# gonewest818/raytrace-clj

Hardware: AMD Instinct MI355X
Metric: Msamples/sec (nx*ny*ns) (higher is better)
Workload: dtype f64; 1 GPU; C3: 1920x1080x256spp Shirley cover scene n=50 (10001 spheres), depth 50, thin-lens camera, seeded counter RNG; accel=bvh; 8x8 tiles dealt round-robin to 1 GPU(s); nx=1920, ny=1080, ns=256, spheres=10001, depth=50, accel=bvh, accel_ran=bvh, frames_in_flight=1, launch_form=one GPU

## Files before the change

include/rtmi.h:

```cpp
#ifndef RTMI_H
#define RTMI_H

#include <stdint.h>

#ifdef __cplusplus
extern "C" {
#endif

#define RTMI_OK 0
#define RTMI_E_ARG (-1)
#define RTMI_E_DEVICE (-2)
#define RTMI_E_UNSUPPORTED (-3)
#define RTMI_E_NOMEM (-4)
#define RTMI_E_STATE (-5)

enum { RTMI_PRIM_SPHERE = 0, RTMI_PRIM_UVSPHERE = 1, RTMI_PRIM_MOVING = 2,
       RTMI_PRIM_RECT_XY = 3, RTMI_PRIM_RECT_XZ = 4, RTMI_PRIM_RECT_YZ = 5, RTMI_PRIM_TRIANGLE = 6,
       RTMI_PRIM_MEDIUM = 7, RTMI_PRIM_BOUNDARY = 16 };
enum { RTMI_XFORM_TRANSLATE = 0, RTMI_XFORM_ROTATE_Y = 1 };
enum { RTMI_MAT_LAMBERTIAN = 0, RTMI_MAT_METAL = 1, RTMI_MAT_DIELECTRIC = 2, RTMI_MAT_DIFFUSE_LIGHT = 3,
       RTMI_MAT_ISOTROPIC = 4  };
enum { RTMI_TEX_CONSTANT = 0, RTMI_TEX_UVGRADIENT = 1, RTMI_TEX_CHECKER = 2,
       RTMI_TEX_PERLIN_NOISE = 3, RTMI_TEX_PERLIN_TURB = 4, RTMI_TEX_MARBLE = 5, RTMI_TEX_FLIP_U = 6, RTMI_TEX_FLIP_V = 7,
       RTMI_TEX_IMAGE = 8 };
// ... 146 lines not shown
int rtmi_last_accel(rtmi_ctx *ctx, int32_t *accel);
int rtmi_last_gather_ms(rtmi_ctx *ctx0, double *ms);

int rtmi_last_traversal_counters(rtmi_ctx *ctx, uint64_t *out_aabb_tests, uint64_t *out_prim_tests);

int rtmi_last_trace_ms(rtmi_ctx *ctx, double *ms, int32_t *launches);
int rtmi_last_reduce_ms(rtmi_ctx *ctx, double *ms, int32_t *launches);

int rtmi_probe_hit(rtmi_scene *scene, int32_t precision, int32_t n, const double *rays, double t_min, double t_max, double *out);
int rtmi_probe_paths(rtmi_scene *scene, int32_t precision, int32_t n, const double *rays, const uint64_t *keys, uint64_t ctr0,
                     int32_t depth, double *out_rgb, uint64_t *out_nseg, double *log, int32_t max_seg, int32_t *out_nlog);
int rtmi_probe_camera(rtmi_scene *scene, int32_t precision, int32_t n, const double *uv, const uint64_t *keys, double *out);
int rtmi_probe_texture(rtmi_scene *scene, int32_t precision, int32_t tex, int32_t n, const double *uvp, double *out);
int rtmi_probe_scatter(rtmi_scene *scene, int32_t precision, int32_t mat, int32_t n, const double *rays, const double *hits,
                       const uint64_t *keys, double *out);
int rtmi_probe_rng(rtmi_ctx *ctx, int32_t precision, uint64_t key, uint64_t d0, int32_t n, uint64_t *out_bits, double *out_real);
uint64_t rtmi_sample_key(uint64_t seed, uint64_t pixel, uint64_t sample);
int rtmi_probe_arith(rtmi_ctx *ctx, int32_t n, const double *abc, double *out);
#define RTMI_PROBE_MATH_SLOTS 12
int rtmi_probe_math2(rtmi_ctx *ctx, int32_t n, const double *abc, double tmin, double tmax, int32_t n_slots, double *out);
int rtmi_probe_math(rtmi_ctx *ctx, int32_t n, const double *abc, double tmin, double tmax, double *out);

int rtmi_test_build_tree(int32_t n, const double *geom, const double *cam, int32_t threads, uint64_t *out_hash, int32_t *out_info, double *out_ms);
int rtmi_test_half_outward(double x, int32_t up);
int rtmi_test_pack_materials(int32_t n_prims, const int32_t *prim_kind, const double *prim_geom, const int32_t *prim_mat,
                             int32_t n_mats, const int32_t *mat_kind, const int32_t *mat_tex, const double *mat_param,
                             int32_t n_tex, const int32_t *tex_kind, const double *tex_param, const int32_t *tex_child,
                             int32_t cam_kind, const double *cam, const int32_t *prim_flip, const int32_t *prim_xform,
                             int32_t n_xforms, const int32_t *xform_kind, const double *xform_param, int32_t through_creation,
                             uint64_t *out_hash, int32_t *out_facts);
int rtmi_test_pack_geometry(int32_t n_prims, const int32_t *prim_kind, const double *prim_geom, const int32_t *prim_mat,
                            int32_t n_mats, const int32_t *mat_kind, const int32_t *mat_tex, const double *mat_param,
                            int32_t n_tex, const int32_t *tex_kind, const double *tex_param, const int32_t *tex_child,
                            int32_t cam_kind, const double *cam, const int32_t *prim_flip, const int32_t *prim_xform,
                            int32_t n_xforms, const int32_t *xform_kind, const double *xform_param, int32_t through_creation, uint64_t *out_hash);
int rtmi_test_refit(int32_t n_prims, const int32_t *prim_kind, const int32_t *prim_flip, const int32_t *prim_xform, int32_t n_xforms, const int32_t *xform_kind,
                    int32_t cam_kind, const double *cam, int32_t n_steps, const double *geoms, const double *xforms,
                    void *out_nodes, int64_t capacity, int64_t *out_bytes, int32_t *out_info, int32_t *out_big,
                    int32_t *out_cells, int64_t cells_capacity, void *out_leaf_box);
int rtmi_test_refit_half(double x, int32_t up);
int rtmi_test_scene_nodes(rtmi_scene *scene, void *buf, int64_t capacity, int64_t *out_bytes);

#ifdef __cplusplus
}
#endif
#endif
// ... 1 lines not shown
```

raytrace_clj_amd/_ffi.py:

```python
import ctypes as C
import os

import numpy as np

try:
    import torch
except ImportError:
    torch = None

_HERE = os.path.dirname(os.path.abspath(__file__))
LIB_PATH = os.environ.get("RTMI_LIB") or os.path.join(_HERE, "lib", "librtmi.so")

SYMBOLS = [
    "rtmi_last_error", "rtmi_backend_name", "rtmi_version", "rtmi_init", "rtmi_shutdown", "rtmi_set_option",
    "rtmi_device_info", "rtmi_scene_create", "rtmi_scene_create_ex", "rtmi_scene_set_perlin", "rtmi_scene_set_images", "rtmi_scene_set_media_calls", "rtmi_scene_set_media_mode", "rtmi_scene_set_media_calls_narrowed", "rtmi_scene_device_bytes", "rtmi_scene_destroy", "rtmi_render", "rtmi_render_device",
    "rtmi_render_tiles_device", "rtmi_local_tiles", "rtmi_assemble_device", "rtmi_last_trace_ms", "rtmi_last_reduce_ms", "rtmi_probe_hit",
    "rtmi_probe_paths", "rtmi_probe_camera", "rtmi_probe_texture", "rtmi_probe_scatter", "rtmi_probe_rng",
    "rtmi_sample_key", "rtmi_test_half_outward", "rtmi_test_build_tree", "rtmi_probe_arith", "rtmi_probe_math", "rtmi_probe_math2", "rtmi_last_traversal_counters",
    "rtmi_scene_clone", "rtmi_render_multi", "rtmi_render_multi_device", "rtmi_last_gather_ms",
    "rtmi_last_gather_path", "rtmi_rccl_probe", "rtmi_stream_idle", "rtmi_last_passes", "rtmi_last_accel",
    "rtmi_render_progressive", "rtmi_render_progressive_device", "rtmi_progressive_samples", "rtmi_progressive_release",
    "rtmi_render_adaptive", "rtmi_render_adaptive_device", "rtmi_adaptive_status", "rtmi_adaptive_active_tiles",
    "rtmi_render_features", "rtmi_render_features_device", "rtmi_denoise", "rtmi_denoise_device",
    "rtmi_adaptive_retire", "rtmi_adaptive_retire_device",
    "rtmi_render_adaptive_tiles_device", "rtmi_assemble_progressive_device", "rtmi_render_multi_adaptive", "rtmi_render_multi_adaptive_device",
    "rtmi_scene_set_camera", "rtmi_scene_set_camera_stream", "rtmi_scene_camera",
    "rtmi_reproject", "rtmi_reproject_device",
    "rtmi_scene_tree_info",
    "rtmi_scene_set_materials", "rtmi_scene_set_materials_stream", "rtmi_test_pack_materials",
    "rtmi_scene_set_geometry", "rtmi_scene_last_refit_ms", "rtmi_test_pack_geometry", "rtmi_test_refit", "rtmi_test_refit_half", "rtmi_test_scene_nodes",
]

F64, F32 = 0, 1
ACCEL_FLAT, ACCEL_BVH = 0, 1
FLAG_TIMING = 1
GATHER_PATHS = {0: "none", 1: "same-device", 2: "peer-copy", 3: "rccl"}
SEG_REC = 12
TILE = 8
PROG_REC = 5
FEATURES = 8
EDIT_STREAM_MAX_BYTES = 32768
# ... 32 lines not shown
    L.rtmi_scene_set_media_mode.argtypes = [vp, i32]
    L.rtmi_scene_set_media_calls_narrowed.argtypes = [vp, i32, vp, vp]
    L.rtmi_scene_device_bytes.argtypes = [vp, C.POINTER(C.c_int64)]
    L.rtmi_scene_destroy.argtypes = [vp]
    L.rtmi_render.argtypes = [vp, i32, i32, i32, i32, u64, i32, i32, i32, i32, i32, vp, vp, vp]
    L.rtmi_render_device.argtypes = [vp, i32, i32, i32, i32, u64, i32, vp, vp, vp, vp]
    L.rtmi_render_tiles_device.argtypes = [vp, i32, i32, i32, i32, u64, i32, i32, i32, vp, vp, vp]
    L.rtmi_local_tiles.argtypes = [i32, i32, i32, i32]
    L.rtmi_local_tiles.restype = i32
    L.rtmi_assemble_device.argtypes = [vp, i32, i32, i32, i32, vp, vp, vp, vp]
    L.rtmi_last_trace_ms.argtypes = [vp, C.POINTER(dbl), C.POINTER(i32)]
    L.rtmi_last_reduce_ms.argtypes = [vp, C.POINTER(dbl), C.POINTER(i32)]
    L.rtmi_probe_hit.argtypes = [vp, i32, i32, vp, dbl, dbl, vp]
    L.rtmi_probe_paths.argtypes = [vp, i32, i32, vp, vp, u64, i32, vp, vp, vp, i32, vp]
    L.rtmi_probe_camera.argtypes = [vp, i32, i32, vp, vp, vp]
    L.rtmi_probe_texture.argtypes = [vp, i32, i32, i32, vp, vp]
    L.rtmi_probe_scatter.argtypes = [vp, i32, i32, i32, vp, vp, vp, vp]
    L.rtmi_probe_rng.argtypes = [vp, i32, u64, u64, i32, vp, vp]
    L.rtmi_sample_key.argtypes = [u64, u64, u64]
    L.rtmi_sample_key.restype = u64
    L.rtmi_probe_arith.argtypes = [vp, i32, vp, vp]
    L.rtmi_test_build_tree.argtypes = [i32, vp, vp, i32, vp, vp, vp]
    L.rtmi_test_half_outward.argtypes = [C.c_double, i32]
    L.rtmi_probe_math.argtypes = [vp, i32, vp, C.c_double, C.c_double, vp]
    L.rtmi_probe_math2.argtypes = [vp, i32, vp, C.c_double, C.c_double, i32, vp]
    L.rtmi_last_traversal_counters.argtypes = [vp, C.POINTER(u64), C.POINTER(u64)]
    L.rtmi_scene_clone.argtypes = [vp, vp, C.POINTER(vp)]
    L.rtmi_render_multi.argtypes = [i32, C.POINTER(vp), i32, i32, i32, i32, u64, i32, vp, vp, vp]
    L.rtmi_render_multi_device.argtypes = [i32, C.POINTER(vp), i32, i32, i32, i32, u64, i32, vp, vp, vp]
    L.rtmi_last_gather_ms.argtypes = [vp, C.POINTER(dbl)]
    L.rtmi_last_gather_path.argtypes = [vp, C.POINTER(i32)]
    L.rtmi_rccl_probe.argtypes = [C.c_char_p]
    L.rtmi_stream_idle.argtypes = [vp, C.POINTER(i32)]
    L.rtmi_last_passes.argtypes = [vp, C.POINTER(i32)]
    L.rtmi_last_accel.argtypes = [vp, C.POINTER(i32)]
    L.rtmi_render_progressive.argtypes = [vp, i32, i32, i32, i32, i32, u64, i32, i32, i32, i32, i32, vp, vp, vp, vp]
    L.rtmi_render_progressive_device.argtypes = [vp, i32, i32, i32, i32, i32, u64, i32, vp, vp, vp, vp, vp]
    L.rtmi_progressive_samples.argtypes = [vp, C.POINTER(i32)]
    L.rtmi_progressive_release.argtypes = [vp]
    L.rtmi_render_adaptive.argtypes = [vp, i32, i32, i32, i32, dbl, i32, u64, i32, i32, i32, i32, i32, vp, vp, vp, vp, vp]
    L.rtmi_render_adaptive_device.argtypes = [vp, i32, i32, i32, i32, dbl, i32, u64, i32, vp, vp, vp, vp, vp, vp]
    L.rtmi_adaptive_status.argtypes = [vp, C.POINTER(i32), C.POINTER(i32), C.POINTER(i64)]
    L.rtmi_adaptive_active_tiles.argtypes = [vp, i32, vp, C.POINTER(i32)]
    L.rtmi_adaptive_retire.argtypes = [vp, i32, i32, vp, dbl, C.POINTER(i32)]
    L.rtmi_adaptive_retire_device.argtypes = [vp, i32, i32, vp, dbl, C.POINTER(i32), vp]
    L.rtmi_render_features.argtypes =[vp, i32, i32, i32, u64, i32, i32, i32, i32, i32, vp, vp]
# ... 46 lines not shown
```

raytrace_clj_amd/csrc/rtmi.hip:

```cpp
#include <hip/hip_runtime.h>
#include <rccl/rccl.h>
#include <dlfcn.h>

#include <algorithm>
#include <atomic>
#include <chrono>
#include <condition_variable>
#include <functional>
#include <thread>
#include <cmath>
#include <cmath>
#include <cstdarg>
#include <cstdio>
#include <cstdlib>
#include <cstring>
#include <array>
#include <map>
#include <mutex>
#include <new>
#include <string>
#include <vector>

#include "rtmi.h"
#include "rtmi_device.h"
// ... 24 lines not shown
#ifndef RTMI_EXT_MIN_WAVES
#define RTMI_EXT_MIN_WAVES RTMI_MIN_WAVES
#endif

struct TraceParams {
    int nx, ny, depth;
    u64 seed;
    int tiles_x;
    int n_local_tiles;
    const int *tile_ids;
    int s_begin, s_count;
    void *samples;
    u64 *counters;
    int prims_per_tile;
    int n_ptiles;
    unsigned *queue;
    unsigned total_items;
    unsigned qblock;
    int suspend_lanes;
    int rx0, ry0, rx1, ry1;
    u64 *trav;
    int susp_off;
    int stash_off;
};
#ifndef RTMI_QUEUE_BLOCK
#define RTMI_QUEUE_BLOCK 256
#endif
#ifndef RTMI_EXT_NO_STASH
#define RTMI_EXT_NO_STASH 0
#endif
#ifndef RTMI_EXT_LDS_STASH
#define RTMI_EXT_LDS_STASH 1
#endif
#ifndef RTMI_STASH
#define RTMI_STASH 1
#endif
constexpr unsigned kQueueBlock = RTMI_QUEUE_BLOCK;

template <typename R> __device__ inline const R *stat4_of(SceneRef sc);
template <typename R> __device__ inline void stage_prims(SceneRef sc, Prim4<R> *lds, int first, int count) {
    for (int i = threadIdx.x; i < count; i += blockDim.x) {
        const R *g = stat4_of<R>(sc) + (size_t)(first + i) * 4;
        Prim4<R> p;
        p.cx = g[0]; p.cy = g[1]; p.cz = g[2]; p.r2 = g[3];
        lds[i] = p;
    }
// ... 118 lines not shown
            __syncthreads();
            stage_prims<R>(sc, lds, first, count);
            __syncthreads();
            if (active) {
                if (VARIANT == SCAN_LDS_PIPE) scan_static_pipe<R, true>(LdsPrims<R>{lds}, count, first, P, a, tmin, best_t, best_i);
                else scan_static<R>(lds, count, first, P, a, tmin, best_t, best_i);
            }
        }
    }
    if (active) {
        if (best_i >= 0) best_i = sc.stat_orig[best_i];
        if (sc.n_moving > 0) {
            int best_orig = best_i >= 0 ? best_i : 0x7fffffff, scan_i = -1;
            scan_moving<R>(sc, P, a, tmin, best_t, scan_i, best_orig);
            if (scan_i >= 0) best_i = best_orig;
        }
    }
}

template <typename R> __device__ inline void start_sample(SceneRef sc, const TraceParams &tp, int i, int j, int s, Path<R> &P) {
    seed_stream(P, sample_key(tp.seed, (u64)j * (u64)tp.nx + (u64)i, (u64)s), 0u);
    const R u = ((R)(float)i + next_uniform(P)) / (R)tp.nx;
    const R v = ((R)(float)j + next_uniform(P)) / (R)tp.ny;
    get_ray<R>(sc, u, v, P);
    P.ar = P.ag = P.ab = R(1);
    P.depth = tp.depth;
}

template <typename R, bool MULTI, int VARIANT, bool EXT = false, bool COUNT = false, bool SLICE = true, int MSEQ = 0, bool LST = false>
__global__ void __launch_bounds__(kTraceBlock, EXT ? ((MSEQ != 0 || COUNT) ? 3 : RTMI_EXT_MIN_WAVES) : RTMI_MIN_WAVES) trace_kernel(ScenePtr scp, TraceParams tp) {
    SceneRef sc = *scp;
    extern __shared__ __attribute__((aligned(16))) char smem[];
    Prim4<R> *lds = reinterpret_cast<Prim4<R> *>(smem);
    const int lane = threadIdx.x & 63;
    if (!MULTI && VARIANT < SCAN_SGPR) stage_prims<R>(sc, lds, 0, sc.n_static);
    __syncthreads();

    const unsigned total_items = tp.total_items;
    unsigned w_cur = 0, w_end = 0;
    Path<R> P;
    P.ox = P.oy = P.oz = P.dx = P.dy = P.dz = P.time = R(0);
    P.ar = P.ag = P.ab = R(0);
    seed_stream(P, 0ull, 0u); P.depth = 0;
    bool alive = false;
    bool exhausted = (total_items == 0);
    unsigned out_item = 0;
    constexpr bool LSTASH = (EXT && RTMI_STASH && RTMI_EXT_LDS_STASH && !RTMI_EXT_NO_STASH) || LST;
    constexpr bool STASH = RTMI_STASH && !(EXT && RTMI_EXT_NO_STASH) && !LSTASH;
    int *const lst = reinterpret_cast<int *>(smem) + tp.stash_off + (threadIdx.x & ~63);
    R st_ox = R(0), st_oy = R(0), st_oz = R(0), st_dx = R(0), st_dy = R(0), st_dz = R(0), st_time = R(0);
    u64 st_rs = 0;
    unsigned st_item = 0xffffffffu;
    unsigned s_head = 64u;
    unsigned nrays = 0;
    unsigned ntrav[2] = {0u, 0u};
    const R tmin = R(0.001), tmax = Real<R>::tmax();
    constexpr bool SLICED = SLICE && VARIANT == SCAN_BVH && !MULTI;
    bool mid = false;

    RTMI_STAMP_DECL
    for (;;) {
        RTMI_PH(PH_LOOP)
        if (LSTASH) {
        for (;;) {
            const u64 dead = __ballot(!alive);
            if (dead == 0) break;
            if (s_head == 64u) {
                if (exhausted) break;
                if (w_cur == w_end) {
                    unsigned base = 0;
                    if (lane == 0) base = atomicAdd(tp.queue, tp.qblock);
                    base = __builtin_amdgcn_readfirstlane(base);
                    if (base >= total_items) { exhausted = true; break; }
                    w_cur = base;
                    w_end = min(base + tp.qblock, total_items);
                }
                const unsigned m = w_cur + (unsigned)lane;
                w_cur += 64u;
                const unsigned chunk = m >> 6;
                const int l = (int)(m & 63u);
                const int tile_local = (int)(chunk / (unsigned)tp.s_count);
                const int s = tp.s_begin + (int)(chunk - (unsigned)tile_local * (unsigned)tp.s_count);
                const int gtile = tp.tile_ids[tile_local];
                const int x = (gtile % tp.tiles_x) * RTMI_TILE + (l & 7);
                const int y = (gtile / tp.tiles_x) * RTMI_TILE + (l >> 3);
                unsigned item = 0xffffffffu;
                if (x >= tp.rx0 && x < tp.rx1 && y >= tp.ry0 && y < tp.ry1) {
                    Path<R> Q;
                    start_sample<R>(sc, tp, x, tp.ny - 1 - y, s, Q);
                    int w0, w1;
                    best_to_words<R>(Q.dx, w0, w1); lst[lane] = w0; lst[kTraceBlock + lane] = w1;
                    best_to_words<R>(Q.dy, w0, w1); lst[2 * kTraceBlock + lane] = w0; lst[3 * kTraceBlock + lane] = w1;
                    best_to_words<R>(Q.dz, w0, w1); lst[4 * kTraceBlock + lane] = w0; lst[5 * kTraceBlock + lane] = w1;
                    best_to_words<R>(Q.time, w0, w1); lst[6 * kTraceBlock + lane] = w0; lst[7 * kTraceBlock + lane] = w1;
                    lst[8 * kTraceBlock + lane] = (int)(unsigned)Q.rs; lst[9 * kTraceBlock + lane] = (int)(unsigned)(Q.rs >> 32);
                    if (!sc.cam_fixed_origin) {
                        best_to_words<R>(Q.ox, w0, w1); lst[11 * kTraceBlock + lane] = w0; lst[12 * kTraceBlock + lane] = w1;
                        best_to_words<R>(Q.oy, w0, w1); lst[13 * kTraceBlock + lane] = w0; lst[14 * kTraceBlock + lane] = w1;
                        best_to_words<R>(Q.oz, w0, w1); lst[15 * kTraceBlock + lane] = w0; lst[16 * kTraceBlock + lane] = w1;
                    }
                    item = m;
                    RTMI_PH(PH_REFILL_GEN)
                }
                lst[10 * kTraceBlock + lane] = (int)item;
                s_head = 0u;
            }
            const unsigned avail = 64u - s_head, nd = (unsigned)__popcll(dead);
            const unsigned rank = (unsigned)__popcll(dead & ((1ull << lane) - 1ull));
            if (!alive && rank < avail) {
                const int e = (int)(s_head + rank);
                const unsigned item = (unsigned)lst[10 * kTraceBlock + e];
                if (item != 0xffffffffu) {
// ... 8 lines not shown
                    P.ar = P.ag = P.ab = R(1);
                    P.depth = tp.depth;
                    out_item = item;
                    alive = true;
                }
            }
            s_head += min(nd, avail);
        }
        } else if (STASH) {
        for (;;) {
            const u64 dead = __ballot(!alive);
            if (dead == 0) break;
            if (s_head == 64u) {
                if (exhausted) break;
                if (w_cur == w_end) {
                    unsigned base = 0;
                    if (lane == 0) base = atomicAdd(tp.queue, tp.qblock);
                    base = __builtin_amdgcn_readfirstlane(base);
                    if (base >= total_items) { exhausted = true; break; }
                    w_cur = base;
                    w_end = min(base + tp.qblock, total_items);
                }
                const unsigned m = w_cur + (unsigned)lane;
                w_cur += 64u;
                const unsigned chunk = m >> 6;
                const int l = (int)(m & 63u);
                const int tile_local = (int)(chunk / (unsigned)tp.s_count);
                const int s = tp.s_begin + (int)(chunk - (unsigned)tile_local * (unsigned)tp.s_count);
                const int gtile = tp.tile_ids[tile_local];
                const int x = (gtile % tp.tiles_x) * RTMI_TILE + (l & 7);
                const int y = (gtile / tp.tiles_x) * RTMI_TILE + (l >> 3);
                st_item = 0xffffffffu;
                if (x >= tp.rx0 && x < tp.rx1 && y >= tp.ry0 && y < tp.ry1) {
                    Path<R> Q;
                    start_sample<R>(sc, tp, x, tp.ny - 1 - y, s, Q);
                    st_ox = Q.ox; st_oy = Q.oy; st_oz = Q.oz; st_dx = Q.dx; st_dy = Q.dy; st_dz = Q.dz; st_time = Q.time; st_rs = Q.rs;
                    st_item = m;
                    RTMI_PH(PH_REFILL_GEN)
                }
                s_head = 0u;
            }
            const unsigned avail = 64u - s_head, nd = (unsigned)__popcll(dead);
            const unsigned rank = (unsigned)__popcll(dead & ((1ull << lane) - 1ull));
            const bool take = !alive && rank < avail;
            const int src = take ? (int)(s_head + rank) : lane;
            R f_ox, f_oy, f_oz;
            if (sc.cam_fixed_origin) { f_ox = (R)sc.cam[0]; f_oy = (R)sc.cam[1]; f_oz = (R)sc.cam[2]; }
            else { f_ox = __shfl(st_ox, src); f_oy = __shfl(st_oy, src); f_oz = __shfl(st_oz, src); }
            const R f_dx = __shfl(st_dx, src), f_dy = __shfl(st_dy, src), f_dz = __shfl(st_dz, src), f_time = __shfl(st_time, src);
            const u64 f_rs = __shfl(st_rs, src);
            const unsigned f_item = __shfl(st_item, src);
            if (take && f_item != 0xffffffffu) {
                P.ox = f_ox; P.oy = f_oy; P.oz = f_oz; P.dx = f_dx; P.dy = f_dy; P.dz = f_dz; P.time = f_time; P.rs = f_rs;
                P.ar = P.ag = P.ab = R(1);
                P.depth = tp.depth;
                out_item = f_item;
                alive = true;
            }
// ... 1067 lines not shown
                                          : (multi ? trace_kernel<R, true, SCAN_LDS_LITERAL> : trace_kernel<R, false, SCAN_LDS_LITERAL>);
        p.lds.bytes = lds_bytes;
    }
    return p;
}

#ifdef RTMI_STAMPS
int report_phase_stamps(rtmi_ctx *c, hipStream_t st) {
    const int grid_trace_dbg = c->last_grid;
    HIP_TRY(hipStreamSynchronize(st));
    unsigned long long h[3 * PH_SLOTS] = {0}, z[3 * PH_SLOTS] = {0};
    HIP_TRY(hipMemcpyFromSymbol(h, HIP_SYMBOL(g_phase), sizeof(h)));
    HIP_TRY(hipMemcpyToSymbol(HIP_SYMBOL(g_phase), z, sizeof(z)));
    {
        static unsigned long long wt[2][4096];
        HIP_TRY(hipMemcpyFromSymbol(wt, HIP_SYMBOL(g_wg_t), sizeof(wt)));
        const int g = std::min(4096, grid_trace_dbg);
        unsigned long long t0 = ~0ull; for (int k = 0; k < g; ++k) t0 = std::min(t0, wt[0][k]);
        std::vector<double> e(g), b(g); for (int k = 0; k < g; ++k) { e[k] = (wt[1][k] - t0) * 1e-5; b[k] = (wt[0][k] - t0) * 1e-5; }
        std::sort(e.begin(), e.end()); std::sort(b.begin(), b.end());
        fprintf(stderr, "[stamps] workgroup start (ms after first): median %.3f max %.3f | end: min %.3f p10 %.3f median %.3f p90 %.3f max %.3f (last pass, %d workgroups)\n",
                b[g / 2], b[g - 1], e[0], e[g / 10], e[g / 2], e[g * 9 / 10], e[g - 1], g);
    }
    static const char *names[PH_N] = {"loop/tail", "refill: generate 64 camera rays", "refill: claim + deal", "bvh: ray setup / resume", "bvh: big primitives (exact)",
                                      "bvh: descent (node visits)", "bvh: leaf exact tests", "bvh: loop control / park", "shade: hit record", "shade: |d| normalise",
                                      "shade: rand-in-unit-sphere", "shade: material record + directions", "shade: texture", "shade: store / rest", "shade: sphere uv", "(stamp calibration)",
                                      "bvh: grid entry / next piece of the walk", "media: chords, draws, log"};
    const double per_stamp = h[2 * PH_SLOTS + PH_CAL] ? (double)h[PH_CAL] / (double)h[2 * PH_SLOTS + PH_CAL] : 0.0;
    double tk[PH_N], lk[PH_N], tot = 0, totl = 0, raw = 0;
    for (int k = 0; k < PH_N; ++k) {
        raw += (double)h[k];
        const double t = (double)h[k], c = std::min(t, per_stamp * (double)h[2 * PH_SLOTS + k]);
        tk[k] = k == PH_CAL ? 0.0 : t - c;
        lk[k] = t > 0 ? (double)h[PH_SLOTS + k] * (tk[k] / t) : 0.0;
        tot += tk[k]; totl += lk[k];
    }
    fprintf(stderr, "[phases] one stamp = %.0f ticks; stamps took %.1f %% of the %.4g wave-ticks of this (diagnostic) launch and are subtracted below\n", per_stamp, 100 * (raw - tot) / raw, raw);
    fprintf(stderr, "[phases] %-36s %8s %8s %10s %10s %12s\n", "phase", "ticks %", "lanes", "masked %", "useful %", "stamps");
    for (int k = 0; k < PH_N; ++k) {
        if (!h[k] || k == PH_CAL) continue;
        const double t = tk[k], l = lk[k];
        fprintf(stderr, "[phases] %-36s %8.2f %8.1f %10.2f %10.2f %12llu\n", names[k], 100 * t / tot, t > 0 ? l / t : 0.0, 100 * (64 * t - l) / (64 * tot), 100 * l / (64 * tot), h[2 * PH_SLOTS + k]);
    }
    fprintf(stderr, "[phases] %-36s %8.2f %8.1f %10.2f %10.2f   (%.4g wave-ticks)\n", "total", 100.0, totl / tot, 100 * (64 * tot - totl) / (64 * tot), 100 * totl / (64 * tot), tot);
    return RTMI_OK;
}
#endif

template <typename F> auto with_real(int precision, F f) { return precision == RTMI_F64 ? f(double{}) : f(float{}); }

// ... 178 lines not shown
    if (rc) return rc;
    c->last_passes = (ns + s_per_pass - 1) / s_per_pass;
    if (!prog && s_per_pass < ns) {
        rc = c->accum.ensure((size_t)n_local * 64 * 3 * sizeof(R));
        if (rc) return rc;
    }
    int ppt, nptiles;
    size_t lds_bytes;
    lds_plan(c, s->dev.n_static, sizeof(R), &ppt, &nptiles, &lds_bytes);
    const TracePlan plan = choose_trace_kernel<R>(s, c, read_launch_knobs(), nptiles > 1, lds_bytes);
    c->last_accel = plan.accel;

    TraceParams tp;
    tp.nx = nx; tp.ny = ny; tp.depth = depth; tp.seed = seed; tp.tiles_x = tiles_x_of(nx);
    tp.n_local_tiles = n_local;
    tp.tile_ids = ad ? reinterpret_cast<const int *>(prog->act_tiles[prog->cur].p) : reinterpret_cast<const int *>(c->tile_ids.p);
    tp.samples = c->samples.p;
    tp.counters = d_counters ? reinterpret_cast<u64 *>(d_counters) : reinterpret_cast<u64 *>(c->counters.p);
    tp.prims_per_tile = (c->scan_variant >= SCAN_SGPR || s->dev.has_ext) ? 0 : ppt; tp.n_ptiles = nptiles;
    tp.queue = reinterpret_cast<unsigned *>(reinterpret_cast<u64 *>(c->counters.p) + 2);
    tp.rx0 = region.x0; tp.ry0 = region.y0; tp.rx1 = region.x1; tp.ry1 = region.y1;
    tp.trav = reinterpret_cast<u64 *>(c->counters.p) + 3;
    tp.suspend_lanes = plan.suspend_lanes; tp.susp_off = plan.lds.susp_off; tp.stash_off = plan.lds.stash_off;
    for (int s_begin = s_first; s_begin < s_end; s_begin += s_per_pass) {
        hipEvent_t e1 = nullptr;
        rc = launch_trace_pass(s, plan, tp, s_begin, std::min(s_per_pass, s_end - s_begin), st, &e1);
        if (!rc) rc = launch_fold<R>(c, tp, ns, s_end, d_tiles_linear, d_counters != nullptr, prog, ad, e1, st);
        if (rc) return rc;
    }
#ifdef RTMI_STAMPS
    rc = report_phase_stamps(c, st);
#endif
    if (!rc && ad)
        HIP_TRY(launch_compact(*prog, nullptr, n_local, -1, tiles_x_of(nx), region, st));
    if (!rc && prog) prog->k = s_end;
    return rc;
}

template <typename R>
int render_tiles_impl(rtmi_scene *s, int nx, int ny, int ns, int depth, uint64_t seed, int first, int stride, const int *rg, void *d_tiles_linear,
                      void *d_counters, hipStream_t st) {
    return render_passes<R>(s, nx, ny, 0, ns, depth, seed, first, stride, rg, d_tiles_linear, d_counters, st, nullptr);
}

int check_render_args(rtmi_scene *s, int nx, int ny, int ns, int depth, int precision) {
    if (!scene_ok(s)) return fail(RTMI_E_STATE, "invalid scene handle");
// ... 45 lines not shown
    std::vector<int> kind((size_t)n, RTMI_PRIM_SPHERE);
    std::vector<BvhBox> wbox((size_t)n);
    std::vector<char> bounded((size_t)n, 0), box_first((size_t)n, 0);
    for (int i = 0; i < n; ++i) {
        const double g[9] = {geom[4 * (size_t)i], geom[4 * (size_t)i + 1], geom[4 * (size_t)i + 2], geom[4 * (size_t)i + 3], 0, 0, 0, 0, 1};
        bounded[(size_t)i] = prim_world_box(RTMI_PRIM_SPHERE, g, nullptr, nullptr, 0, 0, 0.0, 1.0, wbox[(size_t)i]);
    }
    DevScene d{};
    std::vector<int> grid_cells;
    int depth = 0;
    g_build_single.store(threads == 1 ? 1 : 0);
    const double t0 = now_ms();
    const std::vector<float> nodes = build_bvh(d, n, kind.data(), wbox, bounded, cam, true, grid_cells, box_first, knobs, &depth);
    *out_ms = now_ms() - t0;
    g_build_single.store(0);
    uint64_t h = 1469598103934665603ull;
    auto mix = [&](const void *p, size_t bytes) { const unsigned char *q = (const unsigned char *)p; for (size_t k = 0; k < bytes; ++k) { h ^= q[k]; h *= 1099511628211ull; } };
    mix(nodes.data(), nodes.size() * sizeof(float));
    mix(grid_cells.data(), grid_cells.size() * sizeof(int));
    mix(&d.bvh_root, sizeof(int)); mix(&d.grid_tall, sizeof(int)); mix(&d.bvh_node16, sizeof(int));
    *out_hash = h;
    out_info[0] = (int32_t)(nodes.size() / (d.bvh_node16 ? 8 : 16)); out_info[1] = depth; out_info[2] = d.grid_n; out_info[3] = d.n_big;
    return RTMI_OK;
}
RTMI_EXPORT int rtmi_test_half_outward(double x, int32_t up) { return (int)half_outward((float)x, up != 0); }
RTMI_EXPORT const char *rtmi_last_error(void) { return g_err.c_str(); }
RTMI_EXPORT const char *rtmi_backend_name(void) { return "hip-gfx950"; }
RTMI_EXPORT int rtmi_version(void) { return 214; }
RTMI_EXPORT uint64_t rtmi_sample_key(uint64_t seed, uint64_t pixel, uint64_t sample) { return sample_key(seed, pixel, sample); }

RTMI_EXPORT int rtmi_init(int device, uint32_t flags, rtmi_ctx **out_ctx) {
    if (!out_ctx) return fail(RTMI_E_ARG, "out_ctx is NULL");
    *out_ctx = nullptr;
    int ndev = 0;
    if (hipGetDeviceCount(&ndev) != hipSuccess || ndev <= 0) return fail(RTMI_E_DEVICE, "no HIP device visible (this library has no CPU fallback)");
    if (device < 0 || device >= ndev) return fail(RTMI_E_ARG, "device %d out of range (0..%d)", device, ndev - 1);
    HIP_TRY(hipSetDevice(device));
    hipDeviceProp_t prop;
    HIP_TRY(hipGetDeviceProperties(&prop, device));
    if (std::strncmp(prop.gcnArchName, "gfx950", 6) != 0)
        return fail(RTMI_E_DEVICE, "device %d is %s; this library carries gfx950 (MI355X) code objects only", device, prop.gcnArchName);
    rtmi_ctx *c = new (std::nothrow) rtmi_ctx();
    if (!c) return fail(RTMI_E_NOMEM, "out of host memory");
    c->device = device;
    c->flags = flags;
    c->cus = prop.multiProcessorCount;
// ... 2529 lines not shown
```

raytrace_clj_amd/csrc/rtmi_device.h:

```cpp
#pragma once
#include <hip/hip_runtime.h>
#include <stdint.h>

#include "rtmi.h"

namespace rtmi {

typedef unsigned long long u64;

struct DevScene {
    int n_static;
    int n_moving;
    const double *stat_geom;
    const double *stat4_d;
    const float *stat4_f;
    int n_all;
    const float *cull20;
    const double *exact12;
    double cull_t_lo, cull_t_hi;
    const float *bvh_nodes;
    int bvh_root;
    int n_big;
    int big_idx[16];
    int bvh_node16;
// ... 45 lines not shown
    const int *tex_kind;
    const double *tex_param;
    const int *tex_child;
    int cam_kind;
    int cam_fixed_origin;
    double cam[24];
};
typedef const __attribute__((address_space(4))) DevScene &SceneRef;
typedef const __attribute__((address_space(4))) DevScene *ScenePtr;

#define RTMI_GOLD 0x9E3779B97F4A7C15ULL
__host__ __device__ inline u64 mix64(u64 z) {
    z ^= z >> 32; z *= 0xD6E8FEB86659FD93ULL;
    z ^= z >> 32; z *= 0xD6E8FEB86659FD93ULL;
    z ^= z >> 32;
    return z;
}
__host__ __device__ inline u64 sample_key(u64 seed, u64 pix, u64 s) {
    return mix64(mix64(seed ^ (RTMI_GOLD * (pix + 1))) + 0xD1B54A32D192ED03ULL * (s + 1));
}
__host__ __device__ inline u64 draw_bits(u64 key, u64 d) { return mix64(key + RTMI_GOLD * (d + 1)); }

#ifdef RTMI_STAMPS
enum { PH_LOOP = 0, PH_REFILL_GEN, PH_REFILL_DEAL, PH_BVH_SETUP, PH_BIG, PH_DESCENT, PH_LEAF, PH_BVH_POST, PH_HITREC, PH_DNORM, PH_SAMPLER, PH_DIRS, PH_TEXTURE, PH_STORE, PH_UV, PH_CAL, PH_GRID, PH_MEDIA, PH_N };
#define PH_SLOTS 20
__shared__ unsigned long long g_ph[4][3 * PH_SLOTS + 2];
__device__ inline void ph_stamp(int k, unsigned lane_trips = 0, unsigned trips = 0) {
    __builtin_amdgcn_sched_barrier(0);
    unsigned long long t;
    asm volatile("s_memtime %0\n\ts_waitcnt lgkmcnt(0)" : "=s"(t)::"memory");
    const unsigned long long ex = __ballot(1);
    const int w = threadIdx.x >> 6;
    if ((int)(threadIdx.x & 63) == __ffsll((long long)ex) - 1) {
        const unsigned long long dt = t - g_ph[w][3 * PH_SLOTS];
        if (k >= 0) {
            g_ph[w][2 * PH_SLOTS + k] += 1;
            g_ph[w][k] += dt;
            g_ph[w][PH_SLOTS + k] += trips ? dt * (unsigned long long)lane_trips / (unsigned long long)trips : dt * (unsigned long long)__popcll(ex);
        }
        g_ph[w][3 * PH_SLOTS] = t;
    }
    __builtin_amdgcn_sched_barrier(0);
}
#define RTMI_PH(k) ph_stamp(k);
#define RTMI_PH_LANES(k, lt, tr) ph_stamp(k, lt, tr);
#elif defined(RTMI_MARKERS)
#define RTMI_PH(k) asm volatile("; PHASE_END " #k);
#define RTMI_PH_LANES(k, lt, tr) asm volatile("; PHASE_END " #k);
// ... 247 lines not shown
        const u64 sm = kStrideMask[n];
        const u64 mine = pending ? ((acc >> vrank) & sm) : 0ull;
        const int first = mine ? __ffsll((long long)mine) - 1 : 0;
        const int src = mine ? vrank + first : lane;
        const R fx = __shfl(cx, src), fy = __shfl(cy, src), fz = __shfl(cz, src);
        if (pending) {
            const unsigned used = mine ? 3u * (unsigned)(__popcll(sm & ((1ull << first) - 1ull)) + 1) : 3u * (unsigned)K;
            P.rs += RTMI_GOLD * (u64)used;
            P.ctr += used;
            if (mine) { x = fx; y = fy; z = fz; pending = false; }
        }
        RTMI_PH(PH_SAMPLER)
        rem = __ballot(pending);
    }
#else
    if (need) rand_in_unit_sphere(P, x, y, z);
#endif
}

template <typename R> __device__ inline void rand_in_unit_disk(Path<R> &P, R &x, R &y) {
    for (;;) {
        x = next_symmetric(P);
        y = next_symmetric(P);
        if (!(dot3(x, y, R(0), x, y, R(0)) >= R(1.0))) return;
    }
}

template <typename R> __device__ inline void get_ray(SceneRef sc, R s, R t, Path<R> &P) {
    unsigned long long cam_addr = (unsigned long long)(&sc.cam[0]);
    asm volatile("" : "+s"(cam_addr));
    const __attribute__((address_space(4))) double *c = (const __attribute__((address_space(4))) double *)cam_addr;
    const R ox = (R)c[0], oy = (R)c[1], oz = (R)c[2];
    R dx = (((R)c[3] + (R)c[6] * s) + (R)c[9] * t) + (-ox);
    R dy = (((R)c[4] + (R)c[7] * s) + (R)c[10] * t) + (-oy);
    R dz = (((R)c[5] + (R)c[8] * s) + (R)c[11] * t) + (-oz);
    if (sc.cam_kind == RTMI_CAM_PINHOLE) {
        P.ox = ox; P.oy = oy; P.oz = oz; P.dx = dx; P.dy = dy; P.dz = dz; P.time = R(0);
        return;
    }
    const R lens_radius = (R)c[21] / R(2.0);
    R rx, ry;
    rand_in_unit_disk(P, rx, ry);
    rx = lens_radius * rx; ry = lens_radius * ry;
    const R offx = (R)c[12] * rx + (R)c[15] * ry;
    const R offy = (R)c[13] * rx + (R)c[16] * ry;
    const R offz = (R)c[14] * rx + (R)c[17] * ry;
    P.ox = ox + offx; P.oy = oy + offy; P.oz = oz + offz;
    P.dx = dx + (-offx); P.dy = dy + (-offy); P.dz = dz + (-offz);
    const R t0 = (R)c[22], t1 = (R)c[23];
    P.time = t0 + (t1 - t0) * next_uniform(P);
}

template <typename R> __device__ inline int sin_sign(R x) {
    const R s = Real<R>::sin_(x);
    return s < R(0) ? -1 : (s > R(0) ? 1 : 0);
}
template <> __device__ inline int sin_sign<double>(double x) {
    if (x == 0.0) return 0;
    if (!(fabs(x) <= 1.0e5)) { const double s = ::sin(x); return s < 0.0 ? -1 : (s > 0.0 ? 1 : 0); }
    const double k = ::rint(x * 0.3183098861837907);
    double r = ::fma(-k, 3.141592653589793, x);
    r = ::fma(-k, 1.2246467991473532e-16, r);
    const bool odd = ((int)k) & 1;
    return (odd != (r < 0.0)) ? -1 : 1;
}

template <typename R> __device__ inline R perlin_noise(SceneRef sc, R px, R py, R pz) {
    const R fi = (R)::floor((double)px), fj = (R)::floor((double)py), fk = (R)::floor((double)pz);
    const int i = (int)fi, j = (int)fj, k = (int)fk;
    const R u = px - fi, v = py - fj, w = pz - fk;
    const R uu = (u * u) * (R(3.0) - R(2.0) * u), vv = (v * v) * (R(3.0) - R(2.0) * v), ww = (w * w) * (R(3.0) - R(2.0) * w);
    R acc = R(0);
#pragma unroll
// ... 1461 lines not shown
```

raytrace_clj_amd/csrc/scene_build.h:

```cpp
#pragma once
#include <unistd.h>

namespace {

struct BuildKnobs {
    int sah_levels = 1 << 20;
    int sweep_max = 0;
    double min_frac = 0.0;
    bool grid_off = false;
    int grid_side = 0;
    int grid_kmax = 4;
    bool grid_walk = true;
    bool mloc = false;
    int node16 = -1;
    bool box_leaf = false;
    bool small_scan = true;
    bool debug = false;
};
inline BuildKnobs read_build_knobs() {
    BuildKnobs k;
    if (const char *e = std::getenv("RTMI_BVH_SAH_LEVELS")) k.sah_levels = std::atoi(e);
    if (const char *e = std::getenv("RTMI_BVH_SWEEP_MAX")) k.sweep_max = std::atoi(e);
    if (const char *e = std::getenv("RTMI_BVH_MIN_FRAC")) k.min_frac = std::atof(e);
    if (const char *e = std::getenv("RTMI_GRID")) { k.grid_off = e[0] == '0'; k.grid_side = std::atoi(e); }
// ... 609 lines not shown
            const int k = a.tex_kind[t];
            char u = k == RTMI_TEX_IMAGE ? 3 : 0;
            if (k == RTMI_TEX_UVGRADIENT) {
                const double *tp = a.tex_param + (size_t)t * RTMI_TEX_STRIDE;
                bool var_u = false, var_v = false;
                auto same = [&](int x, int y) { return std::memcmp(&tp[x], &tp[y], sizeof(double)) == 0; };
                for (int c = 0; c < 3; ++c) {
                    var_u = var_u || !same(c, 3 + c) || !same(6 + c, 9 + c);
                    var_v = var_v || !same(c, 6 + c) || !same(3 + c, 9 + c);
                }
                u = (char)((var_u ? 1 : 0) | (var_v ? 2 : 0));
            }
            if (k == RTMI_TEX_CHECKER || k == RTMI_TEX_FLIP_U || k == RTMI_TEX_FLIP_V)
                for (int c = 0; c < (k == RTMI_TEX_CHECKER ? 2 : 1); ++c) {
                    const int ch = a.tex_child[2 * (size_t)t + c];
                    if (ch >= 0 && ch < a.n_tex) u |= uses[(size_t)ch];
                }
            if (uses[(size_t)t] != u) { uses[(size_t)t] = u; changed = true; }
        }
    }
    return uses;
}

inline int camera_fixed_origin(int cam_kind, const double *cam) {
    bool fixed = cam_kind == RTMI_CAM_PINHOLE || cam[21] == 0.0;
    for (int k = 0; k < 3; ++k) fixed = fixed && !(cam[k] == 0.0 && std::signbit(cam[k])) && std::isfinite(cam[k]);
    for (int k = 12; k < 18; ++k) fixed = fixed && std::isfinite(cam[k]);
    return fixed ? 1 : 0;
}
inline void camera_shutter(int cam_kind, const double *cam, double &t_lo, double &t_hi) {
    t_lo = cam_kind == RTMI_CAM_THINLENS ? std::min(cam[22], cam[23]) : 0.0;
    t_hi = cam_kind == RTMI_CAM_THINLENS ? std::max(cam[22], cam[23]) : 0.0;
}

PackedMaterials pack_materials(const SceneArrays &a) {
    PackedMaterials M;
    const int n_prims = a.n_prims;
    for (int t = 0; t < a.n_tex; ++t) {
        if (a.tex_kind[t] > RTMI_TEX_CHECKER) M.has_ext = true;
        if (a.tex_kind[t] >= RTMI_TEX_PERLIN_NOISE && a.tex_kind[t] <= RTMI_TEX_MARBLE) M.uses_perlin = true;
        if (a.tex_kind[t] == RTMI_TEX_IMAGE) M.max_image = std::max(M.max_image, (int)a.tex_param[(size_t)t * RTMI_TEX_STRIDE]);
    }
    for (int i = 0; i < n_prims; ++i)
        if (a.mat_kind[a.prim_mat[i]] == RTMI_MAT_ISOTROPIC) M.has_ext = true;
    const std::vector<char> uses = texture_uv_use(a);
    M.prim_mat.assign(a.prim_mat, a.prim_mat + n_prims);
    M.prim_kind.resize((size_t)n_prims);
    for (int i = 0; i < n_prims; ++i) {
        const int kind = a.prim_kind[i] & ~RTMI_PRIM_BOUNDARY;
        M.prim_kind[(size_t)i] = kind;
// ... 262 lines not shown
```

Measured before the change: 7730 Msamples/s.

## Generate camera rays wave-cooperatively with shared lens-disk rejection and cached pixel hash

```diff
diff --git a/include/rtmi.h b/include/rtmi.h
--- a/include/rtmi.h
+++ b/include/rtmi.h
@@ -192,6 +192,7 @@
 int rtmi_probe_math(rtmi_ctx *ctx, int32_t n, const double *abc, double tmin, double tmax, double *out);
 
 int rtmi_test_build_tree(int32_t n, const double *geom, const double *cam, int32_t threads, uint64_t *out_hash, int32_t *out_info, double *out_ms);
+int rtmi_test_camera_fixed(int32_t cam_kind, const double *cam);
 int rtmi_test_half_outward(double x, int32_t up);
 int rtmi_test_pack_materials(int32_t n_prims, const int32_t *prim_kind, const double *prim_geom, const int32_t *prim_mat,
                              int32_t n_mats, const int32_t *mat_kind, const int32_t *mat_tex, const double *mat_param,
diff --git a/raytrace_clj_amd/_ffi.py b/raytrace_clj_amd/_ffi.py
--- a/raytrace_clj_amd/_ffi.py
+++ b/raytrace_clj_amd/_ffi.py
@@ -16,7 +16,7 @@
     "rtmi_device_info", "rtmi_scene_create", "rtmi_scene_create_ex", "rtmi_scene_set_perlin", "rtmi_scene_set_images", "rtmi_scene_set_media_calls", "rtmi_scene_set_media_mode", "rtmi_scene_set_media_calls_narrowed", "rtmi_scene_device_bytes", "rtmi_scene_destroy", "rtmi_render", "rtmi_render_device",
     "rtmi_render_tiles_device", "rtmi_local_tiles", "rtmi_assemble_device", "rtmi_last_trace_ms", "rtmi_last_reduce_ms", "rtmi_probe_hit",
     "rtmi_probe_paths", "rtmi_probe_camera", "rtmi_probe_texture", "rtmi_probe_scatter", "rtmi_probe_rng",
-    "rtmi_sample_key", "rtmi_test_half_outward", "rtmi_test_build_tree", "rtmi_probe_arith", "rtmi_probe_math", "rtmi_probe_math2", "rtmi_last_traversal_counters",
+    "rtmi_sample_key", "rtmi_test_half_outward", "rtmi_test_camera_fixed", "rtmi_test_build_tree", "rtmi_probe_arith", "rtmi_probe_math", "rtmi_probe_math2", "rtmi_last_traversal_counters",
     "rtmi_scene_clone", "rtmi_render_multi", "rtmi_render_multi_device", "rtmi_last_gather_ms",
     "rtmi_last_gather_path", "rtmi_rccl_probe", "rtmi_stream_idle", "rtmi_last_passes", "rtmi_last_accel",
     "rtmi_render_progressive", "rtmi_render_progressive_device", "rtmi_progressive_samples", "rtmi_progressive_release",
@@ -95,6 +95,7 @@
     L.rtmi_probe_arith.argtypes = [vp, i32, vp, vp]
     L.rtmi_test_build_tree.argtypes = [i32, vp, vp, i32, vp, vp, vp]
     L.rtmi_test_half_outward.argtypes = [C.c_double, i32]
+    L.rtmi_test_camera_fixed.argtypes = [i32, vp]
     L.rtmi_probe_math.argtypes = [vp, i32, vp, C.c_double, C.c_double, vp]
     L.rtmi_probe_math2.argtypes = [vp, i32, vp, C.c_double, C.c_double, i32, vp]
     L.rtmi_last_traversal_counters.argtypes = [vp, C.POINTER(u64), C.POINTER(u64)]
diff --git a/raytrace_clj_amd/csrc/rtmi.hip b/raytrace_clj_amd/csrc/rtmi.hip
--- a/raytrace_clj_amd/csrc/rtmi.hip
+++ b/raytrace_clj_amd/csrc/rtmi.hip
@@ -70,6 +70,8 @@
     u64 *trav;
     int susp_off;
     int stash_off;
+    double rnx, rny;
+    int fixed_rays;
 };
 #ifndef RTMI_QUEUE_BLOCK
 #define RTMI_QUEUE_BLOCK 256
@@ -234,9 +236,46 @@
     seed_stream(P, sample_key(tp.seed, (u64)j * (u64)tp.nx + (u64)i, (u64)s), 0u);
     const R u = ((R)(float)i + next_uniform(P)) / (R)tp.nx;
     const R v = ((R)(float)j + next_uniform(P)) / (R)tp.ny;
+    RTMI_PH(PH_GEN_KEY)
     get_ray<R>(sc, u, v, P);
     P.ar = P.ag = P.ab = R(1);
     P.depth = tp.depth;
+}
+
+__device__ inline double pixel_quot(double x, int n, double rn) { return div_const(x, (double)n, rn); }
+__device__ inline float pixel_quot(float x, int n, double) { return x / (float)n; }
+
+#ifndef RTMI_GEN_PLAIN
+#define RTMI_GEN_PLAIN 0
+#endif
+struct GenTile { int tile, x0, y0; u64 hpix; };
+template <typename R, bool KEEP> __device__ inline bool generate_camera_rays(SceneRef sc, const TraceParams &tp, unsigned chunk, int lane, GenTile &g, Path<R> &Q) {
+    const int tile_local = (int)(chunk / (unsigned)tp.s_count);
+    const int s = tp.s_begin + (int)(chunk - (unsigned)tile_local * (unsigned)tp.s_count);
+#if RTMI_GEN_PLAIN
+    const int gtile = tp.tile_ids[tile_local];
+    const int x = (gtile % tp.tiles_x) * RTMI_TILE + (lane & 7), y = (gtile / tp.tiles_x) * RTMI_TILE + (lane >> 3);
+    const bool has = x >= tp.rx0 && x < tp.rx1 && y >= tp.ry0 && y < tp.ry1;
+    if (has) start_sample<R>(sc, tp, x, tp.ny - 1 - y, s, Q);
+    return has;
+#else
+    if (!KEEP || tile_local != g.tile) {
+        const int gtile = tp.tile_ids[tile_local];
+        g.x0 = (gtile % tp.tiles_x) * RTMI_TILE; g.y0 = (gtile / tp.tiles_x) * RTMI_TILE;
+        const int i = g.x0 + (lane & 7), j = tp.ny - 1 - (g.y0 + (lane >> 3));
+        g.hpix = mix64(tp.seed ^ (RTMI_GOLD * ((u64)j * (u64)tp.nx + (u64)i + 1)));
+        g.tile = tile_local;
+    }
+    const int x = g.x0 + (lane & 7), y = g.y0 + (lane >> 3), j = tp.ny - 1 - y;
+    const bool has = x >= tp.rx0 && x < tp.rx1 && y >= tp.ry0 && y < tp.ry1;
+    seed_stream(Q, mix64(g.hpix + 0xD1B54A32D192ED03ULL * ((u64)s + 1)), 0u);
+    const R ju = next_uniform(Q), jv = next_uniform(Q);
+    const R u = pixel_quot((R)(float)x + ju, tp.nx, tp.rnx);
+    const R v = pixel_quot((R)(float)j + jv, tp.ny, tp.rny);
+    RTMI_PH(PH_GEN_KEY)
+    get_ray_wave<R>(sc, tp.fixed_rays != 0, has, u, v, Q);
+    return has;
+#endif
 }
 
 template <typename R, bool MULTI, int VARIANT, bool EXT = false, bool COUNT = false, bool SLICE = true, int MSEQ = 0, bool LST = false>
@@ -264,6 +303,8 @@
     u64 st_rs = 0;
     unsigned st_item = 0xffffffffu;
     unsigned s_head = 64u;
+    constexpr bool KEEP = LST;
+    GenTile gen = {-1, 0, 0, 0ull};
     unsigned nrays = 0;
     unsigned ntrav[2] = {0u, 0u};
     const R tmin = R(0.001), tmax = Real<R>::tmax();
@@ -288,18 +329,11 @@
                     w_end = min(base + tp.qblock, total_items);
                 }
                 const unsigned m = w_cur + (unsigned)lane;
+                Path<R> Q;
+                const bool has = generate_camera_rays<R, KEEP>(sc, tp, w_cur >> 6, lane, gen, Q);
                 w_cur += 64u;
-                const unsigned chunk = m >> 6;
-                const int l = (int)(m & 63u);
-                const int tile_local = (int)(chunk / (unsigned)tp.s_count);
-                const int s = tp.s_begin + (int)(chunk - (unsigned)tile_local * (unsigned)tp.s_count);
-                const int gtile = tp.tile_ids[tile_local];
-                const int x = (gtile % tp.tiles_x) * RTMI_TILE + (l & 7);
-                const int y = (gtile / tp.tiles_x) * RTMI_TILE + (l >> 3);
                 unsigned item = 0xffffffffu;
-                if (x >= tp.rx0 && x < tp.rx1 && y >= tp.ry0 && y < tp.ry1) {
-                    Path<R> Q;
-                    start_sample<R>(sc, tp, x, tp.ny - 1 - y, s, Q);
+                if (has) {
                     int w0, w1;
                     best_to_words<R>(Q.dx, w0, w1); lst[lane] = w0; lst[kTraceBlock + lane] = w1;
                     best_to_words<R>(Q.dy, w0, w1); lst[2 * kTraceBlock + lane] = w0; lst[3 * kTraceBlock + lane] = w1;
@@ -354,18 +388,11 @@
                     w_end = min(base + tp.qblock, total_items);
                 }
                 const unsigned m = w_cur + (unsigned)lane;
+                Path<R> Q;
+                const bool has = generate_camera_rays<R, KEEP>(sc, tp, w_cur >> 6, lane, gen, Q);
                 w_cur += 64u;
-                const unsigned chunk = m >> 6;
-                const int l = (int)(m & 63u);
-                const int tile_local = (int)(chunk / (unsigned)tp.s_count);
-                const int s = tp.s_begin + (int)(chunk - (unsigned)tile_local * (unsigned)tp.s_count);
-                const int gtile = tp.tile_ids[tile_local];
-                const int x = (gtile % tp.tiles_x) * RTMI_TILE + (l & 7);
-                const int y = (gtile / tp.tiles_x) * RTMI_TILE + (l >> 3);
                 st_item = 0xffffffffu;
-                if (x >= tp.rx0 && x < tp.rx1 && y >= tp.ry0 && y < tp.ry1) {
-                    Path<R> Q;
-                    start_sample<R>(sc, tp, x, tp.ny - 1 - y, s, Q);
+                if (has) {
                     st_ox = Q.ox; st_oy = Q.oy; st_oz = Q.oz; st_dx = Q.dx; st_dy = Q.dy; st_dz = Q.dz; st_time = Q.time; st_rs = Q.rs;
                     st_item = m;
                     RTMI_PH(PH_REFILL_GEN)
@@ -1479,10 +1506,11 @@
         fprintf(stderr, "[stamps] workgroup start (ms after first): median %.3f max %.3f | end: min %.3f p10 %.3f median %.3f p90 %.3f max %.3f (last pass, %d workgroups)\n",
                 b[g / 2], b[g - 1], e[0], e[g / 10], e[g / 2], e[g * 9 / 10], e[g - 1], g);
     }
-    static const char *names[PH_N] = {"loop/tail", "refill: generate 64 camera rays", "refill: claim + deal", "bvh: ray setup / resume", "bvh: big primitives (exact)",
+    static const char *names[PH_N] = {"loop/tail", "refill: generate (stash write)", "refill: claim + deal", "bvh: ray setup / resume", "bvh: big primitives (exact)",
                                       "bvh: descent (node visits)", "bvh: leaf exact tests", "bvh: loop control / park", "shade: hit record", "shade: |d| normalise",
                                       "shade: rand-in-unit-sphere", "shade: material record + directions", "shade: texture", "shade: store / rest", "shade: sphere uv", "(stamp calibration)",
-                                      "bvh: grid entry / next piece of the walk", "media: chords, draws, log"};
+                                      "bvh: grid entry / next piece of the walk", "media: chords, draws, log", "generate: key, jitter, u v", "generate: lens disk rounds",
+                                      "generate: camera arithmetic"};
     const double per_stamp = h[2 * PH_SLOTS + PH_CAL] ? (double)h[PH_CAL] / (double)h[2 * PH_SLOTS + PH_CAL] : 0.0;
     double tk[PH_N], lk[PH_N], tot = 0, totl = 0, raw = 0;
     for (int k = 0; k < PH_N; ++k) {
@@ -1707,6 +1735,7 @@
     tp.rx0 = region.x0; tp.ry0 = region.y0; tp.rx1 = region.x1; tp.ry1 = region.y1;
     tp.trav = reinterpret_cast<u64 *>(c->counters.p) + 3;
     tp.suspend_lanes = plan.suspend_lanes; tp.susp_off = plan.lds.susp_off; tp.stash_off = plan.lds.stash_off;
+    tp.rnx = 1.0 / (double)nx; tp.rny = 1.0 / (double)ny; tp.fixed_rays = camera_fixed_rays(s->dev.cam_kind, s->dev.cam_fixed_origin, s->dev.cam);
     for (int s_begin = s_first; s_begin < s_end; s_begin += s_per_pass) {
         hipEvent_t e1 = nullptr;
         rc = launch_trace_pass(s, plan, tp, s_begin, std::min(s_per_pass, s_end - s_begin), st, &e1);
@@ -1798,6 +1827,10 @@
     *out_hash = h;
     out_info[0] = (int32_t)(nodes.size() / (d.bvh_node16 ? 8 : 16)); out_info[1] = depth; out_info[2] = d.grid_n; out_info[3] = d.n_big;
     return RTMI_OK;
+}
+RTMI_EXPORT int rtmi_test_camera_fixed(int32_t cam_kind, const double *cam) {
+    const int o = camera_fixed_origin(cam_kind, cam);
+    return o | (camera_fixed_rays(cam_kind, o, cam) << 1);
 }
 RTMI_EXPORT int rtmi_test_half_outward(double x, int32_t up) { return (int)half_outward((float)x, up != 0); }
 RTMI_EXPORT const char *rtmi_last_error(void) { return g_err.c_str(); }
diff --git a/raytrace_clj_amd/csrc/rtmi_device.h b/raytrace_clj_amd/csrc/rtmi_device.h
--- a/raytrace_clj_amd/csrc/rtmi_device.h
+++ b/raytrace_clj_amd/csrc/rtmi_device.h
@@ -91,8 +91,8 @@
 __host__ __device__ inline u64 draw_bits(u64 key, u64 d) { return mix64(key + RTMI_GOLD * (d + 1)); }
 
 #ifdef RTMI_STAMPS
-enum { PH_LOOP = 0, PH_REFILL_GEN, PH_REFILL_DEAL, PH_BVH_SETUP, PH_BIG, PH_DESCENT, PH_LEAF, PH_BVH_POST, PH_HITREC, PH_DNORM, PH_SAMPLER, PH_DIRS, PH_TEXTURE, PH_STORE, PH_UV, PH_CAL, PH_GRID, PH_MEDIA, PH_N };
-#define PH_SLOTS 20
+enum { PH_LOOP = 0, PH_REFILL_GEN, PH_REFILL_DEAL, PH_BVH_SETUP, PH_BIG, PH_DESCENT, PH_LEAF, PH_BVH_POST, PH_HITREC, PH_DNORM, PH_SAMPLER, PH_DIRS, PH_TEXTURE, PH_STORE, PH_UV, PH_CAL, PH_GRID, PH_MEDIA, PH_GEN_KEY, PH_GEN_DISK, PH_GEN_CAM, PH_N };
+#define PH_SLOTS 24
 __shared__ unsigned long long g_ph[4][3 * PH_SLOTS + 2];
 __device__ inline void ph_stamp(int k, unsigned lane_trips = 0, unsigned trips = 0) {
     __builtin_amdgcn_sched_barrier(0);
@@ -386,7 +386,67 @@
     for (;;) {
         x = next_symmetric(P);
         y = next_symmetric(P);
+        RTMI_PH(PH_GEN_DISK)
         if (!(dot3(x, y, R(0), x, y, R(0)) >= R(1.0))) return;
+    }
+}
+struct CoopSplit { unsigned v[65]; };
+constexpr CoopSplit make_coop_split() {
+    CoopSplit t{};
+    for (unsigned n = 1; n <= 64; ++n) t.v[n] = (65536u / n + 1u) | ((64u / n) << 20);
+    return t;
+}
+constexpr bool coop_split_divides(const CoopSplit &t) {
+    for (unsigned n = 1; n <= 64; ++n)
+        for (unsigned L = 0; L < 64; ++L) if (((L * (t.v[n] & 0xfffffu)) >> 16) != L / n) return false;
+    return true;
+}
+static_assert(coop_split_divides(make_coop_split()), "(L M) >> 16 = L / n");
+__device__ __constant__ const CoopSplit kCoopSplit = make_coop_split();
+#ifndef RTMI_COOP_DISK
+#define RTMI_COOP_DISK 1
+#endif
+template <typename R> __device__ inline void rand_in_unit_disk_wave(Path<R> &P, bool need, bool counts_only, R &x, R &y) {
+    if (!RTMI_COOP_DISK || __ballot(1) != ~0ull) {
+        if (need) rand_in_unit_disk(P, x, y);
+        return;
+    }
+    const int lane = threadIdx.x & 63;
+    bool pending = need;
+    if (pending) {
+        x = next_symmetric(P); y = next_symmetric(P);
+        pending = dot3(x, y, R(0), x, y, R(0)) >= R(1.0);
+    }
+    RTMI_PH(PH_GEN_DISK)
+    u64 rem = __ballot(pending);
+    while (rem) {
+        const int n = __popcll(rem);
+        const unsigned split = kCoopSplit.v[n];
+        const int K = (int)(split >> 20);
+        const int vrank = __popcll(rem & ((1ull << lane) - 1ull));
+        const int dest = pending ? vrank : n + (lane - vrank);
+        const int tbl = __builtin_amdgcn_ds_permute(dest << 2, lane);
+        const int c = (int)(((unsigned)lane * (split & 0xfffffu)) >> 16), j = lane - c * n;
+        const int vic = __builtin_amdgcn_ds_bpermute(j << 2, tbl);
+        const u64 rs_c = __shfl(P.rs, vic) + RTMI_GOLD * (u64)(2 * c);
+        const R cx = Real<R>::symmetric(mix64(rs_c + RTMI_GOLD)), cy = Real<R>::symmetric(mix64(rs_c + 2ull * RTMI_GOLD));
+        const u64 acc = __ballot(c < K && !(dot3(cx, cy, R(0), cx, cy, R(0)) >= R(1.0)));
+        const u64 sm = kStrideMask[n];
+        const u64 mine = pending ? ((acc >> vrank) & sm) : 0ull;
+        const int first = mine ? __ffsll((long long)mine) - 1 : 0;
+        if (!counts_only) {
+            const int src = mine ? vrank + first : lane;
+            const R fx = __shfl(cx, src), fy = __shfl(cy, src);
+            if (mine) { x = fx; y = fy; }
+        }
+        if (pending) {
+            const unsigned used = mine ? 2u * (unsigned)(__popcll(sm & ((1ull << first) - 1ull)) + 1) : 2u * (unsigned)K;
+            P.rs += RTMI_GOLD * (u64)used;
+            P.ctr += used;
+            if (mine) pending = false;
+        }
+        RTMI_PH(PH_GEN_DISK)
+        rem = __ballot(pending);
     }
 }
 
@@ -404,6 +464,7 @@
     }
     const R lens_radius = (R)c[21] / R(2.0);
     R rx, ry;
+    RTMI_PH(PH_GEN_CAM)
     rand_in_unit_disk(P, rx, ry);
     rx = lens_radius * rx; ry = lens_radius * ry;
     const R offx = (R)c[12] * rx + (R)c[15] * ry;
@@ -413,6 +474,36 @@
     P.dx = dx + (-offx); P.dy = dy + (-offy); P.dz = dz + (-offz);
     const R t0 = (R)c[22], t1 = (R)c[23];
     P.time = t0 + (t1 - t0) * next_uniform(P);
+    RTMI_PH(PH_GEN_CAM)
+}
+template <typename R> __device__ inline void get_ray_wave(SceneRef sc, bool fixed_rays, bool has, R s, R t, Path<R> &P) {
+    unsigned long long cam_addr = (unsigned long long)(&sc.cam[0]);
+    asm volatile("" : "+s"(cam_addr));
+    const __attribute__((address_space(4))) double *c = (const __attribute__((address_space(4))) double *)cam_addr;
+    const R ox = (R)c[0], oy = (R)c[1], oz = (R)c[2];
+    R dx = (((R)c[3] + (R)c[6] * s) + (R)c[9] * t) + (-ox);
+    R dy = (((R)c[4] + (R)c[7] * s) + (R)c[10] * t) + (-oy);
+    R dz = (((R)c[5] + (R)c[8] * s) + (R)c[11] * t) + (-oz);
+    if (sc.cam_kind == RTMI_CAM_PINHOLE) {
+        P.ox = ox; P.oy = oy; P.oz = oz; P.dx = dx; P.dy = dy; P.dz = dz; P.time = R(0);
+        return;
+    }
+    RTMI_PH(PH_GEN_CAM)
+    R rx = R(0), ry = R(0);
+    rand_in_unit_disk_wave(P, has, fixed_rays, rx, ry);
+    if (fixed_rays) { P.ox = ox; P.oy = oy; P.oz = oz; P.dx = dx; P.dy = dy; P.dz = dz; }
+    else {
+        const R lens_radius = (R)c[21] / R(2.0);
+        rx = lens_radius * rx; ry = lens_radius * ry;
+        const R offx = (R)c[12] * rx + (R)c[15] * ry;
+        const R offy = (R)c[13] * rx + (R)c[16] * ry;
+        const R offz = (R)c[14] * rx + (R)c[17] * ry;
+        P.ox = ox + offx; P.oy = oy + offy; P.oz = oz + offz;
+        P.dx = dx + (-offx); P.dy = dy + (-offy); P.dz = dz + (-offz);
+    }
+    const R t0 = (R)c[22], t1 = (R)c[23];
+    P.time = t0 + (t1 - t0) * next_uniform(P);
+    RTMI_PH(PH_GEN_CAM)
 }
 
 template <typename R> __device__ inline int sin_sign(R x) {
diff --git a/raytrace_clj_amd/csrc/scene_build.h b/raytrace_clj_amd/csrc/scene_build.h
--- a/raytrace_clj_amd/csrc/scene_build.h
+++ b/raytrace_clj_amd/csrc/scene_build.h
@@ -655,10 +655,16 @@
     return uses;
 }
 
+inline bool camera_component_plain(double v) { return std::isfinite(v) && std::isfinite((float)v) && !(std::signbit(v) && (float)v == 0.0f); }
 inline int camera_fixed_origin(int cam_kind, const double *cam) {
     bool fixed = cam_kind == RTMI_CAM_PINHOLE || cam[21] == 0.0;
-    for (int k = 0; k < 3; ++k) fixed = fixed && !(cam[k] == 0.0 && std::signbit(cam[k])) && std::isfinite(cam[k]);
-    for (int k = 12; k < 18; ++k) fixed = fixed && std::isfinite(cam[k]);
+    for (int k = 0; k < 3; ++k) fixed = fixed && camera_component_plain(cam[k]);
+    for (int k = 12; k < 18; ++k) fixed = fixed && std::isfinite(cam[k]) && std::isfinite((float)cam[k]);
+    return fixed ? 1 : 0;
+}
+inline int camera_fixed_rays(int cam_kind, int fixed_origin, const double *cam) {
+    bool fixed = cam_kind == RTMI_CAM_THINLENS && fixed_origin;
+    for (int k = 3; k < 6; ++k) fixed = fixed && camera_component_plain(cam[k]);
     return fixed ? 1 : 0;
 }
 inline void camera_shutter(int cam_kind, const double *cam, double &t_lo, double &t_hi) {
```

Result: faster. 7821 Msamples/s, median of 6 (+1.2%).
